# polfosol/micro-AES

Hardware: AMD Instinct MI355X
Metric: GiB/s encrypted (AES-128-CTR, 1 GiB buffer per GPU) (higher is better)
Workload: dtype u8; 1 GPU; AES-128-CTR, 1024 MiB per GPU, device-resident, splitmix64 seed 2; parallelism=shard1, bytes_per_gpu=1073741824

## Files before the change

### micro-aes_amd/csrc/uaes_ctr.hip.h

```cpp
#ifndef UAES_CTR_HIP_H_
#define UAES_CTR_HIP_H_

#include "uaes_aes.hip.h"

__device__ __forceinline__ void ctr_words(const uaesk_ctr &c, u64 i, u32 (&w)[4])
{
    if (c.le32) {
        w[0] = c.w0 + (u32)i;
        w[1] = c.w1; w[2] = c.w2; w[3] = c.w3;
        return;
    }
    const u64 v = (c.v0 + i) & 0x00FFFFFFFFFFFFFFull;
    w[0] = c.w0;
    w[1] = c.w1;
    w[2] = bswap32((c.b8 << 24) | (u32)(v >> 32));
    w[3] = bswap32((u32)v);
}

template <int NR, typename LC>
__device__ __forceinline__ uint4 ctr_one_block(const uaesk_rk &rk, const uaesk_ctr &ctr, const uint4 *in, uint4 *out,
                                               u64 i, const LC &lc)
{
    u32 s1[1][4];
    ctr_words(ctr, i, s1[0]);
    enc_blocks<NR, 1>(s1, rk, lc);
    const uint4 d = in[i];
    const uint4 c = make_uint4(d.x ^ s1[0][0], d.y ^ s1[0][1], d.z ^ s1[0][2], d.w ^ s1[0][3]);
    out[i] = c;
    return c;
}

template <int NR, typename LC>
__device__ __forceinline__ void ctr_byte_tail(const uaesk_rk &rk, const uaesk_ctr &ctr, const uint4 *in, uint4 *out,
                                              u64 nfull, u32 rem, const LC &lc)
{
    u32 s1[1][4];
    ctr_words(ctr, nfull, s1[0]);
    enc_blocks<NR, 1>(s1, rk, lc);
    const unsigned char *src = (const unsigned char *)(in + nfull);
    unsigned char *dst = (unsigned char *)(out + nfull);
    for (u32 i = 0; i < rem; ++i)
        dst[i] = src[i] ^ (unsigned char)(s1[0][i >> 2] >> (8 * (i & 3)));
}

template <int NR, typename LC>
__device__ __forceinline__ void ctr_edge_blocks(const uaesk_rk &rk, const uaesk_ctr &ctr, const uint4 *in, uint4 *out,
                                                u64 pre_end, u64 suf, u64 nfull, u32 rem, const LC &lc)
{
    const u64 nedge = pre_end + (nfull - suf);
    const u64 per = (nedge + gridDim.x - 1) / gridDim.x;
    const u64 lo = (u64)blockIdx.x * per;
    u64 hi = lo + per;
    if (hi > nedge) hi = nedge;
    for (u64 e = lo + threadIdx.x; e < hi; e += UAES_WG)
        (void)ctr_one_block<NR>(rk, ctr, in, out, e < pre_end ? e : suf + (e - pre_end), lc);
    if (rem && blockIdx.x == 0 && threadIdx.x == 0) ctr_byte_tail<NR>(rk, ctr, in, out, nfull, rem, lc);
}

#define CTRS_CHUNK 64u

static inline bool ctr_stripes_cross_a(const uaesk_ctr *c, u64 g_lo, u64 n8)
{
    if (!n8) return false;
    const u64 vbase = c->v0 - (c->v0 & 0xffu);
    const u64 first = vbase + (g_lo << 8), last = vbase + ((g_lo + 8 * n8) << 8) - 1;
    return (first >> 40) != (last >> 40);
}

struct CtrGeo {
    u64 first;
    u64 iters;
};

__device__ __forceinline__ u64 ctr_geo_group0(const CtrGeo &g, u64 it)
{
    return g.first + 8ull * ((u64)blockIdx.x + (u64)gridDim.x * it);
}

struct CtrNoFold {
    static constexpr bool of_input = false;
    static constexpr int round_prio = 1;
    static constexpr bool expand2 = true;
    static constexpr bool text_ahead = true;
    __device__ __forceinline__ void operator()(const uint4 &, const uint4 &) const {}
};

template <int NR, typename LC, typename FOLD>
__device__ __forceinline__ void ctr_shared_loop(const uaesk_rk &rk, const uaesk_ctr &ctr, const uint4 *in, uint4 *out,
                                                const CtrGeo &geo, u32 lds_buf, const LC &lc, FOLD &fold)
{
    const u32 wave = threadIdx.x >> 6, lane = threadIdx.x & 63u;
    const u32 p = ((wave & 3u) << 6) | lane;
    const u32 quad = wave >> 2;
    const u32 c0 = (u32)ctr.v0 & 0xffu;
    const u64 vbase = ctr.v0 - c0;
    uint4 *buf = (uint4 *)(uaes_lds + lds_buf);
    const u32 lane_blk = (quad << 8) | p;

    const u32 x15 = ((p << 24) ^ rk.w[3]) & 0xff000000u;
    struct { u32 w[4 * (NR - 2)]; } rkv;
#pragma unroll
    for (int i = 0; i < 4 * (NR - 2); ++i) rkv.w[i] = rk.w[12 + i];
    u32 L0 = 0, L1 = 0, L2 = 0, L3 = 0;
    u32 parity = 0;

    u64 it = 0;
    uint4 d_cur[2] = { make_uint4(0, 0, 0, 0), make_uint4(0, 0, 0, 0) };
    if (FOLD::text_ahead && it < geo.iters) {
        const u64 g0 = ctr_geo_group0(geo, 0);
#pragma unroll
        for (int u = 0; u < 2; ++u) d_cur[u] = (in + (((g0 + 4u * u) << 8) - c0))[lane_blk];
    }

    const u32 lane_byte = lane_blk * 16u;
    typedef u32 u32x4 __attribute__((ext_vector_type(4)));
#define STRIPE_RSRC(p) __builtin_amdgcn_make_buffer_rsrc( \
        (void *)(((u64)(u32)__builtin_amdgcn_readfirstlane((int)((u64)(p) >> 32)) << 32) | \
                 (u64)(u32)__builtin_amdgcn_readfirstlane((int)(u32)(u64)(p))), 0, 0x7fffffff, 0x00020000)
#define TL(k, b, w) tlook_true<k, b>(w, lc)
    if (geo.iters) {
        const u64 v = (vbase + (ctr_geo_group0(geo, 0) << 8)) & 0x00FFFFFFFFFFFFFFull;
        const u32 s0 = ctr.w0 ^ rk.w[0], s1 = ctr.w1 ^ rk.w[1];
        const u32 s2 = bswap32((ctr.b8 << 24) | (u32)(v >> 32)) ^ rk.w[2];
        const u32 A = xor3(TL(0, 0, s0), TL(1, 1, s1), TL(2, 2, s2)) ^ rk.w[4];
        const u32 col0 = A ^ TL(3, 3, x15);
        L0 = TL(0, 0, col0);
        L1 = TL(3, 3, col0);
        L2 = TL(2, 2, col0);
        L3 = TL(1, 1, col0);
    }
    auto refill = [&](u64 it) {
        {
            if (wave == 0) {
                const u32 gi = lane;
                const u64 g = ctr_geo_group0(geo, it + (gi >> 3)) + (gi & 7u);
                const u64 v = (vbase + (g << 8)) & 0x00FFFFFFFFFFFFFFull;
                const u32 s0 = ctr.w0 ^ rk.w[0], s1 = ctr.w1 ^ rk.w[1];
                const u32 s2 = bswap32((ctr.b8 << 24) | (u32)(v >> 32)) ^ rk.w[2];
                const u32 s3 = (bswap32((u32)v) ^ rk.w[3]) & 0x00ffffffu;
                const u32 c1 = xor3(xor3(TL(0, 0, s1), TL(1, 1, s2), TL(2, 2, s3)), TL(3, 3, s0), rk.w[5]);
                const u32 c2 = xor3(xor3(TL(0, 0, s2), TL(1, 1, s3), TL(2, 2, s0)), TL(3, 3, s1), rk.w[6]);
                const u32 c3 = xor3(xor3(TL(0, 0, s3), TL(1, 1, s0), TL(2, 2, s1)), TL(3, 3, s2), rk.w[7]);
                const u32 u0 = xor3(TL(1, 1, c1), TL(2, 2, c2), TL(3, 3, c3)) ^ rk.w[8];
                const u32 u1 = xor3(TL(0, 0, c1), TL(1, 1, c2), TL(2, 2, c3)) ^ rk.w[9];
                const u32 u2 = xor3(TL(0, 0, c2), TL(1, 1, c3), TL(3, 3, c1)) ^ rk.w[10];
                const u32 u3 = xor3(TL(0, 0, c3), TL(2, 2, c1), TL(3, 3, c2)) ^ rk.w[11];
                buf[(parity * CTRS_CHUNK + gi) * 2 + 0] = make_uint4(u0, u1, u2, u3);
            }
            __syncthreads();
        }

    };
    auto body = [&](u64 it, uint4 (&d_cur)[2], uint4 (&d_nxt)[2]) {
        const u64 g0 = ctr_geo_group0(geo, it);
        {
            const u64 gn = FOLD::text_ahead ? ctr_geo_group0(geo, it + 1 < geo.iters ? it + 1 : it) : g0;
            uint4 (&d_ld)[2] = FOLD::text_ahead ? d_nxt : d_cur;
            const __amdgpu_buffer_rsrc_t rin = STRIPE_RSRC(in + ((gn << 8) - c0));
#pragma unroll
            for (int u = 0; u < 2; ++u) {
                const u32x4 v = __builtin_amdgcn_raw_buffer_load_b128(rin, lane_byte, 16384 * u, 0);
                d_ld[u] = make_uint4(v.x, v.y, v.z, v.w);
            }
        }

        u32 s[2][4];
#pragma unroll
        for (int u = 0; u < 2; ++u) {
            const u32 gl = 8u * ((u32)it & 7u) + quad + 4u * u;
            const uint4 uu = buf[(parity * CTRS_CHUNK + gl) * 2 + 0];
            s[u][0] = L0 ^ uu.x; s[u][1] = L1 ^ uu.y; s[u][2] = L2 ^ uu.z; s[u][3] = L3 ^ uu.w;
        }
        enc_rounds_skewed<NR, 3, decltype(rkv), false, LC, FOLD::round_prio>(s[0], s[1], rkv, lc);
        uint4 ct[2];
#pragma unroll
        for (int u = 0; u < 2; ++u) {
            ct[u] = make_uint4(d_cur[u].x ^ s[u][0], d_cur[u].y ^ s[u][1], d_cur[u].z ^ s[u][2], d_cur[u].w ^ s[u][3]);
            (out + (((g0 + 4u * u) << 8) - c0))[lane_blk] = ct[u];
        }
        if (FOLD::of_input) fold(d_cur[0], d_cur[1]); else fold(ct[0], ct[1]);
    };
    uint4 d_a[2], d_b[2];
#pragma unroll
    for (int u = 0; u < 2; ++u) d_a[u] = d_cur[u];
    constexpr bool twice = FOLD::expand2;
    while (it < geo.iters) {
        const u64 end = it + 8 < geo.iters ? it + 8 : geo.iters;
        refill(it);
        if constexpr (twice) {
            for (; it + 2 <= end; it += 2) {
                body(it, d_a, d_b);
                body(it + 1, d_b, d_a);
            }
            if (it < end) { body(it, d_a, d_b); ++it; }
        } else {
            for (; it < end; ++it) {
                body(it, d_a, d_b);
                if (FOLD::text_ahead) {
#pragma unroll
                    for (int u = 0; u < 2; ++u) d_a[u] = d_b[u];
                }
            }
        }
        parity ^= 1u;
    }
#undef TL
#undef STRIPE_RSRC
}

#endif
```

### micro-aes_amd/csrc/uaes_gcm.hip

```cpp
#include <hip/hip_runtime.h>
#include <atomic>
#include <string.h>
#include <stdlib.h>
#include "uaes_ghash.hip.h"

#define GH_PF 4

__global__ __launch_bounds__(GH_PT) void k_ghash_pass(GSrc src, u64 nv, const uint4 *__restrict__ tab8,
                                                     uint4 *__restrict__ accs)
{
    uint4 *T = (uint4 *)uaes_lds;
    for (u32 i = threadIdx.x; i < 4096u; i += GH_PT) T[i] = tab8[i];
    __syncthreads();
    const GhLane gl = gh_lane_setup();

    const u64 stride = (u64)gridDim.x * GH_PT;
    const u64 j = (u64)blockIdx.x * GH_PT + threadIdx.x;
    const u64 steps = (nv + stride - 1) / stride;
    const u64 pad = steps * stride - nv;
    uint4 acc = make_uint4(0, 0, 0, 0);

    u64 k = 0;
    for (; k < steps && (k == 0 || (steps - k) % GH_PF != 0); ++k) {
        const u64 u = k * stride + j;
// ... 174 lines not shown
            u32 w[4];
            gf_to_words(e, w);
            dst[nib_entry(p, v)] = make_uint4(w[0], w[1], w[2], w[3]);
        }
    }
    }
    if (logF && weights_wg) {
        Gf *shY = (Gf *)(uaes_lds + UAES_LDS_ENC + 19456u);
        const u32 wave = threadIdx.x >> 6, lane = threadIdx.x & 63u;
        const u32 fam = wave >> 3, i = wave & 7u;
        if (threadIdx.x < 2) {
            const Gf one = { 0x8000000000000000ull, 0 };
            const u32 base = threadIdx.x ? 15u : 11u;
            shY[16 * threadIdx.x] = one;
#pragma unroll
            for (u32 q = 0; q < 4; ++q) shY[16 * threadIdx.x + (1u << q)] = shPow[base + q];
        }
        __syncthreads();
        {
            const u32 a = i < 1 ? 2u : i < 3 ? 4u : 8u, b = i == 0 || i == 1 || i == 3 ? 1u : (i == 2 || i == 4 ? 2u : 4u);
            if (i < 6) {
                const Gf pr = wave_gfmul(shY[16 * fam + a], shY[16 * fam + b], lane);
                if (lane == 0) shY[16 * fam + a + b] = pr;
            }
        }
        __syncthreads();
        {
            const u32 a = i == 0 ? 4u : i < 4 ? 8u : 12u, b = i < 2 || i == 4 ? 3u : (i == 2 ? 5u : 6u);
            if (i < 5) {
                const Gf pr = wave_gfmul(shY[16 * fam + a], shY[16 * fam + b], lane);
                if (lane == 0) shY[16 * fam + a + b] = pr;
            }
        }
        __syncthreads();
        if (threadIdx.x < 32) {
            u32 w[4];
            gf_to_words(shY[threadIdx.x], w);
            ((uint4 *)(scratch + GS_YLO))[threadIdx.x] = make_uint4(w[0], w[1], w[2], w[3]);
        }
        if (threadIdx.x == 32) *(uint4 *)(scratch + GS_T) = make_uint4(0, 0, 0, 0);
    }
    if (tables_wg && threadIdx.x <= (want_pow64 ? GH_MAXLOG : (maxlog < GH_MAXLOG ? maxlog : GH_MAXLOG))) {
        u32 w[4];
        gf_to_words(shPow[threadIdx.x], w);
        ((uint4 *)(scratch + GS_POW))[threadIdx.x] = make_uint4(w[0], w[1], w[2], w[3]);
    }
}

#define GF_LDS_AES    65536u
#define GF_LDS_BUF    131072u
#define GF_LDS_TOTAL  (GF_LDS_BUF + 2u * CTRS_CHUNK * 32u)

__device__ __forceinline__ uint4 tabmul8_xor_half(uint4 a, uint4 x, const GhLane &gl)
{
    u32 r[4];
    gh_words(a, gl.g, r);
    u32 z[4] = { x.x, x.y, x.z, x.w };
#pragma unroll
    for (int h = 0; h < 2; ++h) {
        u32x4 e[8];
        __builtin_amdgcn_s_setprio(1);
#pragma unroll
        for (int i = 0; i < 8; ++i) {
            const int t = 8 * h + i;
            e[i] = *(lds_cu128 *)(uintptr_t)__builtin_amdgcn_perm(r[t >> 2], gl.so[t >> 2], gl.sel[t & 3]);
        }
        __builtin_amdgcn_s_setprio(0);
#pragma unroll
        for (int w = 0; w < 4; ++w) {
#pragma unroll
            for (int i = 0; i < 8; i += 2) z[w] = xor3(z[w], e[i][w], e[i + 1][w]);
        }
        __builtin_amdgcn_sched_barrier(0);
    }
    return make_uint4(z[0], z[1], z[2], z[3]);
}

template <bool DEC>
struct GhFold {
    static constexpr bool of_input = DEC;
    static constexpr int round_prio = 2;
    static constexpr bool expand2 = false;
    static constexpr bool text_ahead = false;
    uint4 acc[2];
    GhLane gl;
    __device__ __forceinline__ void operator()(const uint4 &c0, const uint4 &c1)
    {
        __builtin_amdgcn_sched_barrier(0);
        acc[0] = tabmul8_xor_half(acc[0], c0, gl);
        acc[1] = tabmul8_xor_half(acc[1], c1, gl);
    }
};



template <int NR, bool DEC>
__global__ __launch_bounds__(UAES_WG) void k_gcm_fused(uaesk_rk rk, uaesk_tables tb, uaesk_ctr ctr,
                                                           const uint4 *in, uint4 *out,
                                                           u64 g_lo, u64 stripes, u64 h1, u64 nfull, u32 rem,
                                                           GSrc front, u64 nfront,
                                                           unsigned char *__restrict__ scratch)
{
    uint4 *T = (uint4 *)uaes_lds;
    const uint4 *tab8 = (const uint4 *)(scratch + GS_TAB8_F);
    for (u32 i = threadIdx.x; i < 4096u; i += UAES_WG) T[i] = tab8[i];
    fill_tables64(tb.te0, GF_LDS_AES);
    const LaneConst2 lc = make_lane_const2(GF_LDS_AES);
    GhFold<DEC> fold;
    fold.gl = gh_lane_setup();

    ctr_edge_blocks<NR>(rk, ctr, in, out, 0, h1, nfull, rem, lc);

    const u32 wave = threadIdx.x >> 6, lane = threadIdx.x & 63u;
    const u32 p = ((wave & 3u) << 6) | lane, quad = wave >> 2;
    const u64 S = 2048ull * gridDim.x;
    const u64 ablk = (front.aad_len + 15) >> 4;
#pragma unroll
    for (int u = 0; u < 2; ++u) {
        const u64 j = 2048ull * blockIdx.x + 256u * (quad + 4u * u) + p;
        fold.acc[u] = make_uint4(0, 0, 0, 0);
        if (j >= S - nfront) {
            const u64 f = j - (S - nfront);
            if (f < ablk) {
                fold.acc[u] = load_vblock_fwd(front, f);
            } else {
                const uint4 d = in[f - ablk];
                const uint4 c = ctr_one_block<NR>(rk, ctr, in, out, f - ablk, lc);
                fold.acc[u] = DEC ? d : c;
            }
        }
    }
    CtrGeo geo;
    geo.first = g_lo;
    geo.iters = stripes / gridDim.x + (blockIdx.x < stripes % gridDim.x ? 1 : 0);
    ctr_shared_loop<NR>(rk, ctr, in, out, geo, GF_LDS_BUF, lc, fold);

    uint4 *TC = (uint4 *)(uaes_lds + GF_LDS_AES);
    uint4 *buf = (uint4 *)uaes_lds;
    {
        static_assert(GT_NTAB * 512u == 3u * UAES_WG, "three table entries per thread");
        const uint4 *g4 = (const uint4 *)(scratch + GS_TAB4);
        const uint4 e0 = g4[threadIdx.x], e1 = g4[threadIdx.x + UAES_WG], e2 = g4[threadIdx.x + 2u * UAES_WG];
        __syncthreads();
        TC[threadIdx.x] = e0; TC[threadIdx.x + UAES_WG] = e1; TC[threadIdx.x + 2u * UAES_WG] = e2;
    }
    __syncthreads();
    uint4 acc = gh_tree<false>(buf, TC, x4(tabmul4(TC, fold.acc[0]), fold.acc[1]), 1024u);
    if (threadIdx.x == 0) buf[GT_BUF - 1] = acc;
    __syncthreads();
    if (threadIdx.x < 64) {
        const u64 last = (u64)blockIdx.x + (u64)gridDim.x * (geo.iters - 1);
        const u32 k = (u32)(stripes - 1 - last);
        const uint4 *yl = (const uint4 *)(scratch + GS_YLO), *zh = (const uint4 *)(scratch + GS_ZHI);
        Gf w = wave_gfmul(gf_from4(yl[k & 15u]), gf_from4(zh[k >> 4]), threadIdx.x);
        w = wave_gfmul(gf_from4(buf[GT_BUF - 1]), w, threadIdx.x);
        if (threadIdx.x == 0) {
            u32 ww[4];
            gf_to_words(w, ww);
            unsigned *t = (unsigned *)(scratch + GS_T);
#pragma unroll
            for (int i = 0; i < 4; ++i) atomicXor(t + i, ww[i]);
        }
    }
}

static int launch_fused(int nr, bool decrypt, hipStream_t st, const uaesk_tables *tb, const uaesk_rk *ek, const uaesk_ctr *c,
// ... 1413 lines not shown
```

### micro-aes_amd/csrc/uaes_kernels.hip

```cpp
#include <hip/hip_runtime.h>
#include <string.h>
#include <mutex>
#include <stdio.h>
#include <stdlib.h>
#include "uaes_aes.hip.h"
#include "uaes_ctr.hip.h"
#include "uaes_gf.h"
#include "uaes_device.h"
#include "uaes_plan.h"
#include <atomic>

#define UAES_U 4

template <int NR, bool DEC, int U>
__global__ __launch_bounds__(UAES_WG) void k_ecb(uaesk_rk rk, uaesk_tables tb,
                                                 const uint4 *in, uint4 *out,
                                                 u64 nfull, u32 rem, u32 padding, uaesk_done done,
                                                 u64 tail_from)
{
    const u64 first = (u64)blockIdx.x * UAES_WG * U;
    uint4 d0[U];
#pragma unroll
    for (int u = 0; u < U; ++u) {
        const u64 i0 = first + (u64)u * UAES_WG + threadIdx.x;
// ... 73 lines not shown
        out[nfull] = make_uint4(s1[0][0], s1[0][1], s1[0][2], s1[0][3]);
    }
    ticket_release(done);
}

template <int NR, int U>
__device__ __forceinline__ void ctr_generic_body(const uaesk_rk &rk, const uaesk_tables &tb, const uaesk_ctr &ctr,
                                                 const uint4 *in, uint4 *out,
                                                 u64 nfull, u32 rem, const int *__restrict__ gate, const uaesk_done &done)
{
    if (gate && *gate != 0) { ticket_release(done); return; }
    const u64 first = (u64)blockIdx.x * UAES_WG * U;
    uint4 d0[U];
#pragma unroll
    for (int u = 0; u < U; ++u) {
        const u64 i0 = first + (u64)u * UAES_WG + threadIdx.x;
        d0[u] = make_uint4(0, 0, 0, 0);
        if (i0 < nfull) d0[u] = in[i0];
    }
    fill_enc_tables(tb.te0);
    const LaneConst lc = make_lane_const();
    const u64 stride = (u64)gridDim.x * UAES_WG * U;

    for (u64 base = first; base < nfull; base += stride) {
        u32 s[U][4];
        uint4 d[U];
        u64 idx[U];
#pragma unroll
        for (int u = 0; u < U; ++u) {
            idx[u] = base + (u64)u * UAES_WG + threadIdx.x;
            d[u] = d0[u];
            if (base != first && idx[u] < nfull) d[u] = in[idx[u]];
            ctr_words(ctr, idx[u], s[u]);
        }
        if (U == 4) {
            enc_blocks_skewed<NR>(s[0], s[1], rk, lc);
            enc_blocks_skewed<NR>(s[2 % U], s[3 % U], rk, lc);
        } else {
            enc_blocks<NR, U>(s, rk, lc);
        }
#pragma unroll
        for (int u = 0; u < U; ++u)
            if (idx[u] < nfull)
                out[idx[u]] = make_uint4(d[u].x ^ s[u][0], d[u].y ^ s[u][1], d[u].z ^ s[u][2], d[u].w ^ s[u][3]);
    }

    if (rem && blockIdx.x == 0 && threadIdx.x == 0) ctr_byte_tail<NR>(rk, ctr, in, out, nfull, rem, lc);
    ticket_release(done);
}

template <int NR, int U>
__global__ __launch_bounds__(UAES_WG, 4) void k_ctr(uaesk_rk rk, uaesk_tables tb, uaesk_ctr ctr,
                                                 const uint4 *in, uint4 *out,
                                                 u64 nfull, u32 rem, const int *__restrict__ gate, uaesk_done done)
{
    ctr_generic_body<NR, U>(rk, tb, ctr, in, out, nfull, rem, gate, done);
}

template <int NR, int U>
__global__ __launch_bounds__(UAES_WG, 4) void k_ctr_ind(const uaesk_rk *__restrict__ rkp, uaesk_tables tb,
                                                     const uaesk_ctr *__restrict__ ctrp,
                                                     const uint4 *in, uint4 *out, u64 nfull, u32 rem)
{
    uaesk_rk rk;
#pragma unroll
    for (int i = 0; i < 4 * (NR + 1); ++i) rk.w[i] = (u32)__builtin_amdgcn_readfirstlane((int)rkp->w[i]);
    uaesk_ctr ctr;
    ctr.w0 = (u32)__builtin_amdgcn_readfirstlane((int)ctrp->w0);
    ctr.w1 = (u32)__builtin_amdgcn_readfirstlane((int)ctrp->w1);
    ctr.w2 = (u32)__builtin_amdgcn_readfirstlane((int)ctrp->w2);
    ctr.w3 = (u32)__builtin_amdgcn_readfirstlane((int)ctrp->w3);
    ctr.b8 = (u32)__builtin_amdgcn_readfirstlane((int)ctrp->b8);
    ctr.le32 = (u32)__builtin_amdgcn_readfirstlane((int)ctrp->le32);
    {
        const u32 lo = (u32)__builtin_amdgcn_readfirstlane((int)(u32)ctrp->v0);
        const u32 hi = (u32)__builtin_amdgcn_readfirstlane((int)(u32)(ctrp->v0 >> 32));
        ctr.v0 = ((u64)hi << 32) | lo;
    }
    const uaesk_done none = { nullptr, nullptr, 0 };
    ctr_generic_body<NR, U>(rk, tb, ctr, in, out, nfull, rem, nullptr, none);
}

#define CTRS_BUF   (UAES_LDS_ENC)
#define UAES_LDS_CTRS (UAES_LDS_ENC + 2u * CTRS_CHUNK * 32u)

template <int NR>
__global__ __launch_bounds__(UAES_WG, 4) void k_ctr_shared2(uaesk_rk rk, uaesk_tables tb, uaesk_ctr ctr,
                                                           const uint4 *in, uint4 *out,
                                                           u64 g_lo, u64 stripes, u64 nfull, u32 rem,
                                                           const int *__restrict__ gate)
{
    if (gate && *gate != 0) return;
    fill_enc_tables(tb.te0);
    const LaneConst lc = make_lane_const();
    const u32 c0 = (u32)ctr.v0 & 0xffu;
    CtrGeo geo;
    geo.first = g_lo;
    geo.iters = stripes / gridDim.x + (blockIdx.x < stripes % gridDim.x ? 1 : 0);
    ctr_edge_blocks<NR>(rk, ctr, in, out, g_lo * 256 - (g_lo ? c0 : 0),
                        (g_lo + 8 * stripes) * 256 - c0, nfull, rem, lc);
    CtrNoFold nofold;
    ctr_shared_loop<NR>(rk, ctr, in, out, geo, CTRS_BUF, lc, nofold);
}

#define XTS_CHUNK 256u

template <int NR, bool PLAIN = false>
__global__ __launch_bounds__(UAES_WG) void k_xts_tweaks(uaesk_rk k2, uaesk_tables tb,
                                                        uint4 raw_tweak, u32 use_raw, u64 first_sector,
                                                        u64 nsectors, u64 chunks_per_sector, u32 serial,
                                                        uint4 *__restrict__ chunk_tw)
{
    LaneConst lc;
    if (PLAIN) {
        for (u32 i = threadIdx.x; i < 256u; i += blockDim.x) ((u32 *)uaes_lds)[i] = tb.te0[i];
        __syncthreads();
    } else {
        fill_enc_tables(tb.te0);
        lc = make_lane_const();
    }
    const u64 stride = (u64)gridDim.x * blockDim.x;
    for (u64 sct = (u64)blockIdx.x * blockDim.x + threadIdx.x; sct < nsectors; sct += stride) {
        u32 s[1][4];
        if (use_raw) {
            s[0][0] = raw_tweak.x; s[0][1] = raw_tweak.y; s[0][2] = raw_tweak.z; s[0][3] = raw_tweak.w;
        } else {
            const u64 id = first_sector + sct;
            s[0][0] = (u32)id; s[0][1] = (u32)(id >> 32); s[0][2] = 0; s[0][3] = 0;
        }
        if (PLAIN) plain_encrypt<NR>((const u32 *)uaes_lds, k2, s[0]); else enc_blocks<NR, 1>(s, k2, lc);
        Tw t;
        t.lo = s[0][0] | ((u64)s[0][1] << 32);
        t.hi = s[0][2] | ((u64)s[0][3] << 32);
        for (u64 c = 0; c < (serial ? chunks_per_sector : 1); ++c) {
            chunk_tw[sct * chunks_per_sector + c] =
                make_uint4((u32)t.lo, (u32)(t.lo >> 32), (u32)t.hi, (u32)(t.hi >> 32));
            t = tw_mul_pow64(tw_mul_pow64(tw_mul_pow64(tw_mul_pow64(t))));
        }
    }
}

#define XTS_POW_N 40
struct XtsPow {
    u64 lo[XTS_POW_N], hi[XTS_POW_N];
};

__device__ __forceinline__ Tw wave_tw_mul(Tw x, u64 elo, u64 ehi, u32 lane)
{
    const Tw xl = tw_mul_pow(x, lane), xh = tw_mul_pow64(xl);
    Tw z = { 0, 0 };
    if ((elo >> lane) & 1) z = xl;
    if ((ehi >> lane) & 1) { z.lo ^= xh.lo; z.hi ^= xh.hi; }
    u32 w[4] = { (u32)z.lo, (u32)(z.lo >> 32), (u32)z.hi, (u32)(z.hi >> 32) };
#pragma unroll
    for (int off = 32; off > 0; off >>= 1) {
#pragma unroll
        for (int q = 0; q < 4; ++q) w[q] ^= __shfl_xor(w[q], off, 64);
    }
    z.lo = w[0] | ((u64)w[1] << 32);
    z.hi = w[2] | ((u64)w[3] << 32);
    return z;
}

__global__ __launch_bounds__(UAES_WG) void k_xts_expand(XtsPow pw, u64 nsectors, u64 chunks_per_sector,
                                                        uint4 *__restrict__ chunk_tw)
{
    const u32 lane = threadIdx.x & 63u;
    const u64 groups = (chunks_per_sector + 63) / 64;
    const u64 nwaves = (u64)gridDim.x * (UAES_WG / 64);
    for (u64 w = (u64)blockIdx.x * (UAES_WG / 64) + (threadIdx.x >> 6); w < nsectors * groups; w += nwaves) {
        const u64 sct = w / groups, r = w - sct * groups;
        const uint4 t0 = chunk_tw[sct * chunks_per_sector];
        Tw t;
        t.lo = t0.x | ((u64)t0.y << 32);
        t.hi = t0.z | ((u64)t0.w << 32);
        for (u32 i = 0; i < XTS_POW_N; ++i)
            if ((r >> i) & 1) t = wave_tw_mul(t, pw.lo[i], pw.hi[i], lane);
        t = tw_mul_a256(t, lane);
        const u64 c = r * 64 + lane;
        if (c != 0 && c < chunks_per_sector)
            chunk_tw[sct * chunks_per_sector + c] =
                make_uint4((u32)t.lo, (u32)(t.lo >> 32), (u32)t.hi, (u32)(t.hi >> 32));
    }
}

// ... 360 lines not shown
        if (row_encrypt<10>(row_pick(pt, L.c), L) != row_pick(ct, L.c)) bad |= 2048;
    }
    if (bad) atomicOr(result, bad);
}

int uaesk_cus()
{
    static volatile int seen[16];
    int dev = 0;
    hipDeviceProp_t p;
    if (hipGetDevice(&dev) != hipSuccess) { (void)hipGetLastError(); return 0; }
    const bool kept = dev >= 0 && dev < 16;
    if (kept && seen[dev]) return seen[dev];
    if (hipGetDeviceProperties(&p, dev) != hipSuccess) { (void)hipGetLastError(); return 0; }
    if (kept) seen[dev] = p.multiProcessorCount;
    return p.multiProcessorCount;
}

static unsigned grid_for(u64 work_items, u64 per_wg, unsigned cus = uaesk_cus_or_256())
{
    u64 want = (work_items + per_wg - 1) / per_wg;
    if (want < 1) want = 1;
    const u64 cap = cus;
    return (unsigned)(want < cap ? want : cap);
}

hipError_t uaesk_want_lds(const void *kern, unsigned bytes)
{
    enum { SLOTS = 512, PROBE = 16 };
    static const void *volatile seen[16][SLOTS];
    int dev = 0;
    if (hipGetDevice(&dev) != hipSuccess || dev < 0 || dev >= 16) dev = 0;
    const unsigned h = (unsigned)(((uintptr_t)kern >> 3) * 2654435761u) >> 16;
    int free_slot = -1;
    for (int i = 0; i < PROBE; ++i) {
        const unsigned s = (h + i) % SLOTS;
        const void *v = seen[dev][s];
        if (v == kern) return hipSuccess;
        if (!v) { free_slot = (int)s; break; }
    }
    hipError_t e = hipFuncSetAttribute(kern, hipFuncAttributeMaxDynamicSharedMemorySize, (int)bytes);
    if (e == hipSuccess && free_slot >= 0) seen[dev][free_slot] = kern;
    return e;
}

static std::atomic<unsigned> g_plan_disabled{ ~0u };
extern "C" unsigned uaesk_plan_disabled(void)
{
    unsigned m = g_plan_disabled.load(std::memory_order_relaxed);
    if (m == ~0u) {
        const char *e = getenv("UAES_PLAN_DISABLE");
        m = (e && *e) ? (unsigned)strtoul(e, nullptr, 0) & 0x7fffffffu : 0u;
        g_plan_disabled.store(m, std::memory_order_relaxed);
    }
    return m;
}
extern "C" void uaesk_plan_disable(unsigned mask) { g_plan_disabled.store(mask & 0x7fffffffu, std::memory_order_relaxed); }
bool uaesk_arr_on(int id) { return !((uaesk_plan_disabled() >> id) & 1u); }

extern "C" const char *uaesk_arrangement_name(int id)
{
    static const char *const names[UAES_ARR_COUNT] = {
        "ecb.single", "ecb.tiled", "ctr.single", "ctr.quad", "ctr.striped", "xts.small", "xts.packed", "xts.bulk",
        "gcm.small", "gcm.chunks", "gcm.twophase", "gcm.striped", "gcm.levels", "ocb.small", "ocb.runs",
        "siv.small", "siv.chunks", "siv.levels" };
    return id >= 0 && id < UAES_ARR_COUNT ? names[id] : "?";
}

static bool short_text(u64 nblocks, unsigned cus = uaesk_cus_or_256())
{
    return grid_for(nblocks, (u64)UAES_WG * UAES_U, cus) * 2 <= cus;
}

static uaes_plan plan_ecb(u64 items)
{
    uaes_plan p = { UAES_ARR_ECB_TILED, 1, 0, 0 };
    const unsigned cus = uaesk_cus_or_256();
    if (short_text(items, cus) && uaesk_arr_on(UAES_ARR_ECB_SINGLE)) { p.arrangement = UAES_ARR_ECB_SINGLE; p.grid = grid_for(items, UAES_WG, cus); }
    else p.grid = grid_for(items, (u64)UAES_WG * UAES_U, cus);
    return p;
}

#define CTR_TAIL_PCT 80u
static uaes_plan plan_ctr(const uaesk_ctr *ctr, size_t len, u64 *g_lo_out, u64 *n8_out)
{
    const u64 nfull = len / 16, nblocks = (len + 15) / 16;
    uaes_plan p = { UAES_ARR_CTR_QUAD, 1, 0, 0 };
    const unsigned grid = uaesk_cus_or_256();
    if (!ctr->le32 && uaesk_arr_on(UAES_ARR_CTR_STRIPED)) {
        const u32 c0 = (u32)ctr->v0 & 0xffu;
        const u64 g_lo = c0 ? 1 : 0, groups = (c0 + nfull) / 256;
        u64 n8 = groups > g_lo ? (groups - g_lo) / 8 : 0;
        if (n8 >= (u64)grid) {
            const u64 r = n8 % grid;
            if (r && n8 > grid && r * 100 < (u64)grid * CTR_TAIL_PCT) n8 -= r;
            p.arrangement = UAES_ARR_CTR_STRIPED; p.grid = grid;
            if (ctr_stripes_cross_a(ctr, g_lo, n8)) p.launches = 2;
            if (g_lo_out) *g_lo_out = g_lo;
            if (n8_out) *n8_out = n8;
            return p;
        }
    }
    if (short_text(nblocks, grid) && uaesk_arr_on(UAES_ARR_CTR_SINGLE)) { p.arrangement = UAES_ARR_CTR_SINGLE; p.grid = grid_for(nblocks, UAES_WG, grid); }
    else p.grid = grid_for(nblocks, (u64)UAES_WG * UAES_U, grid);
    return p;
}

template <int NR, bool DEC>
static int launch_ecb(hipStream_t st, const uaesk_tables *tb, const uaesk_rk *keys,
                      const void *in, void *out, size_t nfull, unsigned rem, unsigned padding)
{
    const unsigned lds = DEC ? UAES_LDS_DEC : UAES_LDS_ENC;
    const u64 items = nfull + ((rem || padding) ? 1 : 0);
    const uaesk_done done = uaesk_ticket_take();
    const uaes_plan pl = plan_ecb(items);
    if (pl.arrangement == UAES_ARR_ECB_SINGLE)
        return uaesk_launch(k_ecb<NR, DEC, 1>, pl.grid, UAES_WG, lds, st, *keys, *tb, in, out, nfull, rem, padding, done, nfull);
    const u64 tile = (u64)UAES_WG * UAES_U, per_round = tile * pl.grid;
    const u64 rounds = (u64)nfull / per_round, left = (u64)nfull - rounds * per_round;
    const u64 tail_from = (rounds && left && left * 100 < per_round * 80) ? rounds * per_round : (u64)nfull;
    return uaesk_launch(k_ecb<NR, DEC, UAES_U>, pl.grid, UAES_WG, lds, st, *keys, *tb, in, out, nfull, rem, padding, done, tail_from);
}

extern "C" int uaesk_ecb(void *stream, const uaesk_tables *tb, int nr, const uaesk_rk *keys,
                         int decrypt, const void *in, void *out, size_t nfull, unsigned rem, unsigned padding)
{
    if (decrypt) padding = 0;
    if (nfull == 0 && rem == 0 && padding == 0) return 0;
    if (padding > 2) return (int)hipErrorInvalidValue;
    if (decrypt) rem = 0;
    DISPATCH_NR(nr, return with_bool(decrypt, [&](auto D) {
        return launch_ecb<NR, decltype(D)::value>(S(stream), tb, keys, in, out, nfull, rem, padding); }));
    return 0;
}

template <int NR, int U>
static int launch_ctr_u(hipStream_t st, const uaesk_tables *tb, const uaesk_rk *ek, const uaesk_ctr *ctr,
                        const void *in, void *out, size_t len, const int *gate)
{
    const u64 nfull = len / 16;
    const u32 rem = (u32)(len % 16);
    const unsigned grid = grid_for(nfull + (rem ? 1 : 0), (u64)UAES_WG * U);
    uaesk_done done = { nullptr, nullptr, 0 };
    if (!gate) done = uaesk_ticket_take();
    return uaesk_launch(k_ctr<NR, U>, grid, UAES_WG, UAES_LDS_ENC, st, *ek, *tb, *ctr, in, out, nfull, rem, gate, done);
}

template <int NR>
static int launch_ctr_striped(hipStream_t st, const uaesk_tables *tb, const uaesk_rk *ek, const uaesk_ctr *ctr,
                              const void *in, void *out, size_t len, const int *gate, unsigned grid, u64 g_lo, u64 n8)
{
    return uaesk_launch(k_ctr_shared2<NR>, grid, UAES_WG, UAES_LDS_CTRS, st, *ek, *tb, *ctr, in, out, g_lo, n8, len / 16,
                        len % 16, gate);
}

template <int NR>
static int launch_ctr(hipStream_t st, const uaesk_tables *tb, const uaesk_rk *ek, const uaesk_ctr *ctr,
                      const void *in, void *out, size_t len, const int *gate)
{
    u64 g_lo = 0, n8 = 0;
    const uaes_plan pl = plan_ctr(ctr, len, &g_lo, &n8);
    if (pl.arrangement == UAES_ARR_CTR_SINGLE) return launch_ctr_u<NR, 1>(st, tb, ek, ctr, in, out, len, gate);
    if (pl.arrangement == UAES_ARR_CTR_QUAD) return launch_ctr_u<NR, UAES_U>(st, tb, ek, ctr, in, out, len, gate);
    if (pl.launches == 2) {
        const u64 nb = ((u64)1 << 40) - (ctr->v0 & (((u64)1 << 40) - 1));
        if (nb == 0 || nb >= len / 16) return launch_ctr_u<NR, UAES_U>(st, tb, ek, ctr, in, out, len, gate);
        uaesk_ctr second = *ctr;
        second.v0 = (ctr->v0 + nb) & 0x00FFFFFFFFFFFFFFull;
        int rc = launch_ctr<NR>(st, tb, ek, ctr, in, out, (size_t)(nb * 16), gate);
        if (rc) return rc;
        return launch_ctr<NR>(st, tb, ek, &second, (const unsigned char *)in + nb * 16, (unsigned char *)out + nb * 16,
                              len - (size_t)(nb * 16), gate);
    }
    return launch_ctr_striped<NR>(st, tb, ek, ctr, in, out, len, gate, pl.grid, g_lo, n8);
}

template <int NR, int U>
static int launch_ctr_ind_u(hipStream_t st, const uaesk_tables *tb, const uaesk_rk *d_rk, const uaesk_ctr *d_ctr,
                            const void *in, void *out, size_t len)
{
    const u64 nfull = len / 16;
    const u32 rem = (u32)(len % 16);
    const unsigned grid = grid_for(nfull + (rem ? 1 : 0), (u64)UAES_WG * U);
    return uaesk_launch(k_ctr_ind<NR, U>, grid, UAES_WG, UAES_LDS_ENC, st, d_rk, *tb, d_ctr, in, out, nfull, rem);
}

extern "C" int uaesk_ctr_xcrypt_ind(void *stream, const uaesk_tables *tb, int nr, const uaesk_rk *d_rk,
                                    const uaesk_ctr *d_ctr, const void *in, void *out, size_t len)
{
    if (len == 0) return 0;
    if (short_text((len + 15) / 16)) { DISPATCH_NR(nr, return (launch_ctr_ind_u<NR, 1>(S(stream), tb, d_rk, d_ctr, in, out, len))); }
    else                             { DISPATCH_NR(nr, return (launch_ctr_ind_u<NR, 4>(S(stream), tb, d_rk, d_ctr, in, out, len))); }
    return 0;
}

extern "C" int uaesk_ctr_xcrypt(void *stream, const uaesk_tables *tb, int nr, const uaesk_rk *ek,
                                const uaesk_ctr *ctr, const void *in, void *out, size_t len,
                                const int *gate)
{
    if (len == 0) return 0;
    DISPATCH_NR(nr, return (launch_ctr<NR>(S(stream), tb, ek, ctr, in, out, len, gate)));
    return 0;
}

#define XTS_SERIAL_CPS 128u

static const XtsPow *xts_pow_table()
{
    static XtsPow tab;
    static std::once_flag once;
    std::call_once(once, [] {
        Tw e = { 1, 0 };
        for (int i = 0; i < 256; ++i) e = tw_mul_pow64(e);
        for (int i = 0; i < XTS_POW_N; ++i) {
            tab.lo[i] = e.lo; tab.hi[i] = e.hi;
            Tw a = e, acc = { 0, 0 };
            for (int b = 0; b < 128; ++b) {
                if (((b < 64 ? e.lo : e.hi) >> (b & 63)) & 1) { acc.lo ^= a.lo; acc.hi ^= a.hi; }
                a = tw_mul_pow(a, 1);
            }
            e = acc;
        }
    });
    return &tab;
}

static void xts_geometry(size_t sector_bytes, u64 *main_blocks, u32 *rem, u64 *cps)
{
    const u32 r = (u32)(sector_bytes % 16);
    const u64 whole = sector_bytes / 16;
    const u64 mb = whole - (r ? 1 : 0);
    u64 c = (whole + XTS_CHUNK - 1) / XTS_CHUNK;
    if (c == 0) c = 1;
    *main_blocks = mb; *rem = r; *cps = c;
}

extern "C" size_t uaesk_xts_scratch_bytes(size_t sector_bytes, size_t nsectors)
{
    u64 mb, cps; u32 r;
    xts_geometry(sector_bytes, &mb, &r, &cps);
    return (size_t)(cps * nsectors * 16);
}

static uaes_plan plan_xts(size_t sector_bytes, size_t nsectors, bool explicit_tweak)
{
    u64 mb, cps; u32 r;
    xts_geometry(sector_bytes, &mb, &r, &cps);
    uaes_plan p = { UAES_ARR_XTS_BULK, 0, 0, 0 };
    const bool one_unit = nsectors == 1 && mb > 0 && cps <= 2ull * XTS_SMALL_CHUNKS;
    const bool few_units = nsectors > 1 && !explicit_tweak && r == 0 && mb > 0 &&
                           (u64)nsectors * ((mb + 63) / 64) <= 4ull * XTS_SMALL_CHUNKS;
    if ((one_unit || few_units) && uaesk_arr_on(UAES_ARR_XTS_SMALL)) {
        p.arrangement = UAES_ARR_XTS_SMALL; p.launches = r ? 2 : 1;
        p.grid = grid_for((u64)nsectors * ((mb + 63) / 64), UAES_WG / 64);
        return p;
    }
    const bool serial = cps <= XTS_SERIAL_CPS;
// ... 114 lines not shown
extern "C" int uaesk_ticket_disarm(void)
{
    const int still = g_armed.flag != nullptr || g_unused;
    g_armed.flag = nullptr;
    g_unused = 0;
    return still;
}

void uaesk_ticket_unused() { g_unused = 1; }

uaesk_done uaesk_ticket_take()
{
    const uaesk_done d = g_armed;
    g_armed.flag = nullptr;
    return d;
}

__global__ __launch_bounds__(64) void k_ticket(unsigned *flag, unsigned seq, const unsigned *src, unsigned *dst, unsigned nwords)
{
    if (threadIdx.x < nwords) dst[threadIdx.x] = src[threadIdx.x];
    __threadfence_system();
    __syncthreads();
    if (threadIdx.x == 0) __hip_atomic_store(flag, seq, __ATOMIC_RELEASE, __HIP_MEMORY_SCOPE_SYSTEM);
}

extern "C" int uaesk_ticket(void *stream, void *pinned_flag, unsigned seq, const void *d_src, void *pinned_dst, unsigned nbytes)
{
    if (nbytes > 64u || (nbytes & 3u)) return (int)hipErrorInvalidValue;
    return uaesk_launch(k_ticket, 1, 64, 0, S(stream), pinned_flag, seq, d_src, pinned_dst, nbytes / 4u);
}

__global__ __launch_bounds__(64) void k_clock_probe(unsigned long long *out, unsigned long long ticks)
{
    const unsigned long long r0 = wall_clock64();
    const unsigned long long c0 = __builtin_readcyclecounter();
    unsigned long long r1 = r0;
    while (r1 - r0 < ticks) {
        __builtin_amdgcn_s_sleep(32);
        r1 = wall_clock64();
    }
    const unsigned long long c1 = __builtin_readcyclecounter();
    if (threadIdx.x == 0) { out[0] = c1 - c0; out[1] = r1 - r0; }
}

extern "C" int uaesk_clock_probe(void *stream, void *d_out16, unsigned long long ticks_100mhz)
{
    return uaesk_launch(k_clock_probe, 1, 64, 0, S(stream), d_out16, ticks_100mhz);
}

extern "C" int uaesk_selftest(void *stream, const uaesk_tables *tb, const uaesk_rk *ek128,
                              const uaesk_rk *dk128, unsigned *d_result)
{
    return uaesk_launch(k_selftest, 2, UAES_WG, UAES_LDS_ENC, S(stream), *ek128, *dk128, *tb, d_result);
}

int uaesk_plan_gcm(int dir, size_t len, size_t aad_len, unsigned flags, const uint8_t *j0, uaes_plan *p);
int uaesk_plan_siv(int dir, size_t len, size_t aad_len, unsigned flags, uaes_plan *p);
int uaesk_plan_ocb(int dir, size_t len, size_t aad_len, uaes_plan *p);

extern "C" int uaesk_plan(int mode, int dir, size_t a, size_t b, unsigned flags, uaes_plan *p)
{
    return uaesk_plan_at(mode, dir, a, b, flags, nullptr, p);
}

extern "C" int uaesk_plan_at(int mode, int dir, size_t a, size_t b, unsigned flags, const uint8_t *counter16, uaes_plan *p)
{
    if (!p) return (int)hipErrorInvalidValue;
    switch (mode) {
    case UAES_PLAN_ECB:
        *p = plan_ecb((u64)((a + 15) / 16));
        return 0;
    case UAES_PLAN_CTR: {
        uaesk_ctr c;
        memset(&c, 0, sizeof c);
        if (counter16) {
            memcpy(&c.w0, counter16, 4);
            memcpy(&c.w1, counter16 + 4, 4);
            c.b8 = counter16[8];
            for (int i = 9; i < 16; ++i) c.v0 = (c.v0 << 8) | counter16[i];
        } else {
            c.v0 = 1;
        }
        c.le32 = (flags >> 3) & 1u;
        *p = plan_ctr(&c, a, nullptr, nullptr);
        return 0;
    }
    case UAES_PLAN_XTS:
        if (a < 16 || b == 0) return (int)hipErrorInvalidValue;
        *p = plan_xts(a, b, (flags >> 1) & 1u);
        return 0;
    case UAES_PLAN_GCM: return uaesk_plan_gcm(dir, a, b, flags, counter16, p);
    case UAES_PLAN_SIV: return uaesk_plan_siv(dir, a, b, flags, p);
    case UAES_PLAN_OCB: return uaesk_plan_ocb(dir, a, b, p);
    default: return (int)hipErrorInvalidValue;
    }
}
```

Baseline: 1580 GiB/s.

## Align CTR striped kernel to buffer start and write ciphertext with streaming stores

The striped CTR kernel now starts its stripes at block 0 of the buffer instead of at a 256-counter group boundary. Per-lane counter low bytes are rotated, and when the start counter is not group-aligned an extra LDS slot per iteration carries the higher-group precomputed state. This makes the global loads and stores aligned to the buffer start. Ciphertext is written with inline-asm global stores carrying an sc1 cache hint, the first plaintext loads are issued before the table fill, and edge blocks move after the main loop. It adds LDS slots and a second refill wave, and relies on hand-written asm and changed planner arithmetic.

```diff
diff --git a/micro-aes_amd/csrc/uaes_ctr.hip.h b/micro-aes_amd/csrc/uaes_ctr.hip.h
--- a/micro-aes_amd/csrc/uaes_ctr.hip.h
+++ b/micro-aes_amd/csrc/uaes_ctr.hip.h
@@ -59,6 +59,12 @@
 
 #define CTRS_CHUNK 64u
 
+static inline bool ctr_blocks_cross_a(const uaesk_ctr *c, u64 b_lo, u64 b_hi)
+{
+    if (b_hi <= b_lo) return false;
+    const u64 first = c->v0 + b_lo, last = c->v0 + b_hi - 1;
+    return (first >> 40) != (last >> 40);
+}
 static inline bool ctr_stripes_cross_a(const uaesk_ctr *c, u64 g_lo, u64 n8)
 {
     if (!n8) return false;
@@ -82,20 +88,46 @@
     static constexpr int round_prio = 1;
     static constexpr bool expand2 = true;
     static constexpr bool text_ahead = true;
+    static constexpr bool aligned = true;
+    static constexpr bool write_through = true;
     __device__ __forceinline__ void operator()(const uint4 &, const uint4 &) const {}
 };
 
+#define CTRS_SLOTS(aligned) ((aligned) ? CTRS_CHUNK + CTRS_CHUNK / 8u : CTRS_CHUNK)
+
+template <typename FOLD>
+__device__ __forceinline__ u64 ctr_geo_block0(const uaesk_ctr &ctr, const CtrGeo &g, u64 it)
+{
+    return (ctr_geo_group0(g, it) << 8) - (FOLD::aligned ? 0u : (u32)ctr.v0 & 0xffu);
+}
+
+template <typename FOLD>
+__device__ __forceinline__ void ctr_first_text(const uaesk_ctr &ctr, const uint4 *in, const CtrGeo &geo, uint4 (&d)[2])
+{
+    d[0] = d[1] = make_uint4(0, 0, 0, 0);
+    if (FOLD::text_ahead && geo.iters) {
+#pragma unroll
+        for (int u = 0; u < 2; ++u) d[u] = (in + ctr_geo_block0<FOLD>(ctr, geo, 0) + 1024u * u)[threadIdx.x];
+    }
+}
+
 template <int NR, typename LC, typename FOLD>
 __device__ __forceinline__ void ctr_shared_loop(const uaesk_rk &rk, const uaesk_ctr &ctr, const uint4 *in, uint4 *out,
-                                                const CtrGeo &geo, u32 lds_buf, const LC &lc, FOLD &fold)
-{
+                                                const CtrGeo &geo, u32 lds_buf, const LC &lc, FOLD &fold,
+                                                const uint4 (&d0)[2])
+{
+    constexpr bool aligned = FOLD::aligned;
+    constexpr u32 slots = CTRS_SLOTS(aligned), per_it = slots / 8u;
     const u32 wave = threadIdx.x >> 6, lane = threadIdx.x & 63u;
-    const u32 p = ((wave & 3u) << 6) | lane;
+    const u32 r = ((wave & 3u) << 6) | lane;
     const u32 quad = wave >> 2;
     const u32 c0 = (u32)ctr.v0 & 0xffu;
+    const u32 p = aligned ? (c0 + r) & 0xffu : r;
+    const u32 carry = aligned ? (c0 + r) >> 8 : 0u;
     const u64 vbase = ctr.v0 - c0;
     uint4 *buf = (uint4 *)(uaes_lds + lds_buf);
-    const u32 lane_blk = (quad << 8) | p;
+    const u32 lane_blk = (quad << 8) | r;
+    const u32 lane_u = lds_buf + (quad + carry) * 32u;
 
     const u32 x15 = ((p << 24) ^ rk.w[3]) & 0xff000000u;
     struct { u32 w[4 * (NR - 2)]; } rkv;
@@ -105,18 +137,12 @@
     u32 parity = 0;
 
     u64 it = 0;
-    uint4 d_cur[2] = { make_uint4(0, 0, 0, 0), make_uint4(0, 0, 0, 0) };
-    if (FOLD::text_ahead && it < geo.iters) {
-        const u64 g0 = ctr_geo_group0(geo, 0);
-#pragma unroll
-        for (int u = 0; u < 2; ++u) d_cur[u] = (in + (((g0 + 4u * u) << 8) - c0))[lane_blk];
-    }
 
     const u32 lane_byte = lane_blk * 16u;
     typedef u32 u32x4 __attribute__((ext_vector_type(4)));
-#define STRIPE_RSRC(p) __builtin_amdgcn_make_buffer_rsrc( \
-        (void *)(((u64)(u32)__builtin_amdgcn_readfirstlane((int)((u64)(p) >> 32)) << 32) | \
-                 (u64)(u32)__builtin_amdgcn_readfirstlane((int)(u32)(u64)(p))), 0, 0x7fffffff, 0x00020000)
+#define UNIFORM_PTR(p) (((u64)(u32)__builtin_amdgcn_readfirstlane((int)((u64)(p) >> 32)) << 32) | \
+                        (u64)(u32)__builtin_amdgcn_readfirstlane((int)(u32)(u64)(p)))
+#define STRIPE_RSRC(p) __builtin_amdgcn_make_buffer_rsrc((void *)UNIFORM_PTR(p), 0, 0x7fffffff, 0x00020000)
 #define TL(k, b, w) tlook_true<k, b>(w, lc)
     if (geo.iters) {
         const u64 v = (vbase + (ctr_geo_group0(geo, 0) << 8)) & 0x00FFFFFFFFFFFFFFull;
@@ -129,34 +155,31 @@
         L2 = TL(2, 2, col0);
         L3 = TL(1, 1, col0);
     }
+    auto u_entry = [&](u64 g, u32 slot) {
+        const u64 v = (vbase + (g << 8)) & 0x00FFFFFFFFFFFFFFull;
+        const u32 s0 = ctr.w0 ^ rk.w[0], s1 = ctr.w1 ^ rk.w[1];
+        const u32 s2 = bswap32((ctr.b8 << 24) | (u32)(v >> 32)) ^ rk.w[2];
+        const u32 s3 = (bswap32((u32)v) ^ rk.w[3]) & 0x00ffffffu;
+        const u32 c1 = xor3(xor3(TL(0, 0, s1), TL(1, 1, s2), TL(2, 2, s3)), TL(3, 3, s0), rk.w[5]);
+        const u32 c2 = xor3(xor3(TL(0, 0, s2), TL(1, 1, s3), TL(2, 2, s0)), TL(3, 3, s1), rk.w[6]);
+        const u32 c3 = xor3(xor3(TL(0, 0, s3), TL(1, 1, s0), TL(2, 2, s1)), TL(3, 3, s2), rk.w[7]);
+        const u32 u0 = xor3(TL(1, 1, c1), TL(2, 2, c2), TL(3, 3, c3)) ^ rk.w[8];
+        const u32 u1 = xor3(TL(0, 0, c1), TL(1, 1, c2), TL(2, 2, c3)) ^ rk.w[9];
+        const u32 u2 = xor3(TL(0, 0, c2), TL(1, 1, c3), TL(3, 3, c1)) ^ rk.w[10];
+        const u32 u3 = xor3(TL(0, 0, c3), TL(2, 2, c1), TL(3, 3, c2)) ^ rk.w[11];
+        buf[(parity * slots + slot) * 2 + 0] = make_uint4(u0, u1, u2, u3);
+    };
     auto refill = [&](u64 it) {
-        {
-            if (wave == 0) {
-                const u32 gi = lane;
-                const u64 g = ctr_geo_group0(geo, it + (gi >> 3)) + (gi & 7u);
-                const u64 v = (vbase + (g << 8)) & 0x00FFFFFFFFFFFFFFull;
-                const u32 s0 = ctr.w0 ^ rk.w[0], s1 = ctr.w1 ^ rk.w[1];
-                const u32 s2 = bswap32((ctr.b8 << 24) | (u32)(v >> 32)) ^ rk.w[2];
-                const u32 s3 = (bswap32((u32)v) ^ rk.w[3]) & 0x00ffffffu;
-                const u32 c1 = xor3(xor3(TL(0, 0, s1), TL(1, 1, s2), TL(2, 2, s3)), TL(3, 3, s0), rk.w[5]);
-                const u32 c2 = xor3(xor3(TL(0, 0, s2), TL(1, 1, s3), TL(2, 2, s0)), TL(3, 3, s1), rk.w[6]);
-                const u32 c3 = xor3(xor3(TL(0, 0, s3), TL(1, 1, s0), TL(2, 2, s1)), TL(3, 3, s2), rk.w[7]);
-                const u32 u0 = xor3(TL(1, 1, c1), TL(2, 2, c2), TL(3, 3, c3)) ^ rk.w[8];
-                const u32 u1 = xor3(TL(0, 0, c1), TL(1, 1, c2), TL(2, 2, c3)) ^ rk.w[9];
-                const u32 u2 = xor3(TL(0, 0, c2), TL(1, 1, c3), TL(3, 3, c1)) ^ rk.w[10];
-                const u32 u3 = xor3(TL(0, 0, c3), TL(2, 2, c1), TL(3, 3, c2)) ^ rk.w[11];
-                buf[(parity * CTRS_CHUNK + gi) * 2 + 0] = make_uint4(u0, u1, u2, u3);
-            }
-            __syncthreads();
-        }
-
+        if (wave == 0) u_entry(ctr_geo_group0(geo, it + (lane >> 3)) + (lane & 7u), per_it * (lane >> 3) + (lane & 7u));
+        if (aligned && c0 != 0 && wave == 1 && lane < 8u) u_entry(ctr_geo_group0(geo, it + lane) + 8u, per_it * lane + 8u);
+        __syncthreads();
     };
     auto body = [&](u64 it, uint4 (&d_cur)[2], uint4 (&d_nxt)[2]) {
-        const u64 g0 = ctr_geo_group0(geo, it);
+        const u64 b0 = ctr_geo_block0<FOLD>(ctr, geo, it);
         {
-            const u64 gn = FOLD::text_ahead ? ctr_geo_group0(geo, it + 1 < geo.iters ? it + 1 : it) : g0;
+            const u64 bn = FOLD::text_ahead ? ctr_geo_block0<FOLD>(ctr, geo, it + 1 < geo.iters ? it + 1 : it) : b0;
             uint4 (&d_ld)[2] = FOLD::text_ahead ? d_nxt : d_cur;
-            const __amdgpu_buffer_rsrc_t rin = STRIPE_RSRC(in + ((gn << 8) - c0));
+            const __amdgpu_buffer_rsrc_t rin = STRIPE_RSRC(in + bn);
 #pragma unroll
             for (int u = 0; u < 2; ++u) {
                 const u32x4 v = __builtin_amdgcn_raw_buffer_load_b128(rin, lane_byte, 16384 * u, 0);
@@ -167,8 +190,13 @@
         u32 s[2][4];
 #pragma unroll
         for (int u = 0; u < 2; ++u) {
-            const u32 gl = 8u * ((u32)it & 7u) + quad + 4u * u;
-            const uint4 uu = buf[(parity * CTRS_CHUNK + gl) * 2 + 0];
+            uint4 uu;
+            if constexpr (aligned) {
+                uu = *(const uint4 *)(uaes_lds + lane_u + (parity * slots + per_it * ((u32)it & 7u) + 4u * u) * 32u);
+            } else {
+                const u32 gl = 8u * ((u32)it & 7u) + quad + 4u * u;
+                uu = buf[(parity * slots + gl) * 2 + 0];
+            }
             s[u][0] = L0 ^ uu.x; s[u][1] = L1 ^ uu.y; s[u][2] = L2 ^ uu.z; s[u][3] = L3 ^ uu.w;
         }
         enc_rounds_skewed<NR, 3, decltype(rkv), false, LC, FOLD::round_prio>(s[0], s[1], rkv, lc);
@@ -176,13 +204,19 @@
 #pragma unroll
         for (int u = 0; u < 2; ++u) {
             ct[u] = make_uint4(d_cur[u].x ^ s[u][0], d_cur[u].y ^ s[u][1], d_cur[u].z ^ s[u][2], d_cur[u].w ^ s[u][3]);
-            (out + (((g0 + 4u * u) << 8) - c0))[lane_blk] = ct[u];
+            if constexpr (FOLD::write_through) {
+                const u64 ob = UNIFORM_PTR(out + b0 + 1024u * u);
+                const u32x4 cv = { ct[u].x, ct[u].y, ct[u].z, ct[u].w };
+                asm volatile("global_store_dwordx4 %0, %1, %2 sc1\n\ts_nop 0" :: "v"(lane_byte), "v"(cv), "s"(ob) : "memory");
+            } else {
+                (out + b0 + 1024u * u)[lane_blk] = ct[u];
+            }
         }
         if (FOLD::of_input) fold(d_cur[0], d_cur[1]); else fold(ct[0], ct[1]);
     };
     uint4 d_a[2], d_b[2];
 #pragma unroll
-    for (int u = 0; u < 2; ++u) d_a[u] = d_cur[u];
+    for (int u = 0; u < 2; ++u) d_a[u] = d0[u];
     constexpr bool twice = FOLD::expand2;
     while (it < geo.iters) {
         const u64 end = it + 8 < geo.iters ? it + 8 : geo.iters;
@@ -206,6 +240,16 @@
     }
 #undef TL
 #undef STRIPE_RSRC
+#undef UNIFORM_PTR
+}
+
+template <int NR, typename LC, typename FOLD>
+__device__ __forceinline__ void ctr_shared_loop(const uaesk_rk &rk, const uaesk_ctr &ctr, const uint4 *in, uint4 *out,
+                                                const CtrGeo &geo, u32 lds_buf, const LC &lc, FOLD &fold)
+{
+    uint4 d0[2];
+    ctr_first_text<FOLD>(ctr, in, geo, d0);
+    ctr_shared_loop<NR>(rk, ctr, in, out, geo, lds_buf, lc, fold, d0);
 }
 
 #endif
diff --git a/micro-aes_amd/csrc/uaes_gcm.hip b/micro-aes_amd/csrc/uaes_gcm.hip
--- a/micro-aes_amd/csrc/uaes_gcm.hip
+++ b/micro-aes_amd/csrc/uaes_gcm.hip
@@ -280,6 +280,8 @@
     static constexpr int round_prio = 2;
     static constexpr bool expand2 = false;
     static constexpr bool text_ahead = false;
+    static constexpr bool aligned = false;
+    static constexpr bool write_through = false;
     uint4 acc[2];
     GhLane gl;
     __device__ __forceinline__ void operator()(const uint4 &c0, const uint4 &c1)
diff --git a/micro-aes_amd/csrc/uaes_kernels.hip b/micro-aes_amd/csrc/uaes_kernels.hip
--- a/micro-aes_amd/csrc/uaes_kernels.hip
+++ b/micro-aes_amd/csrc/uaes_kernels.hip
@@ -179,25 +179,25 @@
 }
 
 #define CTRS_BUF   (UAES_LDS_ENC)
-#define UAES_LDS_CTRS (UAES_LDS_ENC + 2u * CTRS_CHUNK * 32u)
+#define UAES_LDS_CTRS (UAES_LDS_ENC + 2u * CTRS_SLOTS(CtrNoFold::aligned) * 32u)
 
 template <int NR>
 __global__ __launch_bounds__(UAES_WG, 4) void k_ctr_shared2(uaesk_rk rk, uaesk_tables tb, uaesk_ctr ctr,
                                                            const uint4 *in, uint4 *out,
-                                                           u64 g_lo, u64 stripes, u64 nfull, u32 rem,
+                                                           u64 stripes, u64 nfull, u32 rem,
                                                            const int *__restrict__ gate)
 {
     if (gate && *gate != 0) return;
+    CtrGeo geo;
+    geo.first = 0;
+    geo.iters = stripes / gridDim.x + (blockIdx.x < stripes % gridDim.x ? 1 : 0);
+    uint4 d0[2];
+    ctr_first_text<CtrNoFold>(ctr, in, geo, d0);
     fill_enc_tables(tb.te0);
     const LaneConst lc = make_lane_const();
-    const u32 c0 = (u32)ctr.v0 & 0xffu;
-    CtrGeo geo;
-    geo.first = g_lo;
-    geo.iters = stripes / gridDim.x + (blockIdx.x < stripes % gridDim.x ? 1 : 0);
-    ctr_edge_blocks<NR>(rk, ctr, in, out, g_lo * 256 - (g_lo ? c0 : 0),
-                        (g_lo + 8 * stripes) * 256 - c0, nfull, rem, lc);
     CtrNoFold nofold;
-    ctr_shared_loop<NR>(rk, ctr, in, out, geo, CTRS_BUF, lc, nofold);
+    ctr_shared_loop<NR>(rk, ctr, in, out, geo, CTRS_BUF, lc, nofold, d0);
+    ctr_edge_blocks<NR>(rk, ctr, in, out, 0, 2048 * stripes, nfull, rem, lc);
 }
 
 #define XTS_CHUNK 256u
@@ -724,7 +724,7 @@
 }
 
 #define CTR_TAIL_PCT 80u
-static uaes_plan plan_ctr(const uaesk_ctr *ctr, size_t len, u64 *g_lo_out, u64 *n8_out)
+static uaes_plan plan_ctr(const uaesk_ctr *ctr, size_t len, u64 *n8_out)
 {
     const u64 nfull = len / 16, nblocks = (len + 15) / 16;
     uaes_plan p = { UAES_ARR_CTR_QUAD, 1, 0, 0 };
@@ -732,13 +732,12 @@
     if (!ctr->le32 && uaesk_arr_on(UAES_ARR_CTR_STRIPED)) {
         const u32 c0 = (u32)ctr->v0 & 0xffu;
         const u64 g_lo = c0 ? 1 : 0, groups = (c0 + nfull) / 256;
-        u64 n8 = groups > g_lo ? (groups - g_lo) / 8 : 0;
-        if (n8 >= (u64)grid) {
+        if (groups >= g_lo + 8 * (u64)grid) {
+            u64 n8 = nfull / 2048;
             const u64 r = n8 % grid;
             if (r && n8 > grid && r * 100 < (u64)grid * CTR_TAIL_PCT) n8 -= r;
             p.arrangement = UAES_ARR_CTR_STRIPED; p.grid = grid;
-            if (ctr_stripes_cross_a(ctr, g_lo, n8)) p.launches = 2;
-            if (g_lo_out) *g_lo_out = g_lo;
+            if (ctr_blocks_cross_a(ctr, 0, 2048 * n8)) p.launches = 2;
             if (n8_out) *n8_out = n8;
             return p;
         }
@@ -790,9 +789,9 @@
 
 template <int NR>
 static int launch_ctr_striped(hipStream_t st, const uaesk_tables *tb, const uaesk_rk *ek, const uaesk_ctr *ctr,
-                              const void *in, void *out, size_t len, const int *gate, unsigned grid, u64 g_lo, u64 n8)
-{
-    return uaesk_launch(k_ctr_shared2<NR>, grid, UAES_WG, UAES_LDS_CTRS, st, *ek, *tb, *ctr, in, out, g_lo, n8, len / 16,
+                              const void *in, void *out, size_t len, const int *gate, unsigned grid, u64 n8)
+{
+    return uaesk_launch(k_ctr_shared2<NR>, grid, UAES_WG, UAES_LDS_CTRS, st, *ek, *tb, *ctr, in, out, n8, len / 16,
                         len % 16, gate);
 }
 
@@ -800,8 +799,8 @@
 static int launch_ctr(hipStream_t st, const uaesk_tables *tb, const uaesk_rk *ek, const uaesk_ctr *ctr,
                       const void *in, void *out, size_t len, const int *gate)
 {
-    u64 g_lo = 0, n8 = 0;
-    const uaes_plan pl = plan_ctr(ctr, len, &g_lo, &n8);
+    u64 n8 = 0;
+    const uaes_plan pl = plan_ctr(ctr, len, &n8);
     if (pl.arrangement == UAES_ARR_CTR_SINGLE) return launch_ctr_u<NR, 1>(st, tb, ek, ctr, in, out, len, gate);
     if (pl.arrangement == UAES_ARR_CTR_QUAD) return launch_ctr_u<NR, UAES_U>(st, tb, ek, ctr, in, out, len, gate);
     if (pl.launches == 2) {
@@ -814,7 +813,7 @@
         return launch_ctr<NR>(st, tb, ek, &second, (const unsigned char *)in + nb * 16, (unsigned char *)out + nb * 16,
                               len - (size_t)(nb * 16), gate);
     }
-    return launch_ctr_striped<NR>(st, tb, ek, ctr, in, out, len, gate, pl.grid, g_lo, n8);
+    return launch_ctr_striped<NR>(st, tb, ek, ctr, in, out, len, gate, pl.grid, n8);
 }
 
 template <int NR, int U>
@@ -1095,7 +1094,7 @@
             c.v0 = 1;
         }
         c.le32 = (flags >> 3) & 1u;
-        *p = plan_ctr(&c, a, nullptr, nullptr);
+        *p = plan_ctr(&c, a, nullptr);
         return 0;
     }
     case UAES_PLAN_XTS:
```

Result: faster. 1598 GiB/s, median of 6 (+1.2%).
